# boguszjelinski/taxidispatcher

Measured on AMD Instinct MI355X. Metric: NxN assignments/sec, higher is better.
Workload: dtype int32; 1 GPU; g1 N=16384: device cost write (4N^2 B) + exact assignment, total checked == optimum; n=16384, parallelism=single GPU

## Files before the change

taxidispatcher_amd/csrc/td_assign.hip:

```cpp
#include <dlfcn.h>
#include <limits.h>
#include <stdlib.h>

#include <type_traits>

#include "td_common.h"

using namespace td;

namespace {

template <typename CT>
struct Tr;
template <>
struct Tr<uint8_t> {
    using PT = int32_t;
    static constexpr int E = 16;
    static constexpr uint32_t SENT = 0xFFu;
    static constexpr int64_t LIMIT = 254;
    static constexpr int32_t BIG = 1 << 28;
    static constexpr int32_t KMAX = INT32_MAX;
};
template <>
struct Tr<uint16_t> {
// ... 3094 lines not shown
            k_compress_tr<8><<<dim3((n + 63) / 64, (n + 511) / 512), 256, 0, c.stream>>>(n, npad, sv.d_cost, (uint32_t *)sv.cc.p, 0, colmin, colmax, ctl);
        else
            k_compress_tr<1><<<dim3((n + 63) / 64, (n + 63) / 64), 256, 0, c.stream>>>(n, npad, sv.d_cost, (uint32_t *)sv.cc.p, 0, colmin, colmax, ctl);
        k_tr_finish<<<(n + 255) / 256, 256, 0, c.stream>>>(n, 0, colmin, colmax, (int32_t *)sv.rowmin.p, (int *)sv.rconst.p, ctl, esc_raw,
                                                           cells8 ? 1 : 0, nosync ? (long long)assumed_range : -1ll);
    }
    TD_HIP(hipGetLastError());
    if (nosync) {
        *fits = true;
        sv.nconst = -1;
        sv.nchunks = nchunks;
        sv.npad = npad;
        return TD_OK;
    }
    TD_HIP(hipMemcpyAsync(c.pinned, ctl, 8 * sizeof(int), hipMemcpyDeviceToHost, c.stream));
    TD_HIP(hipStreamSynchronize(c.stream));
    const int *h = (const int *)c.pinned;
    *range = (int64_t)(((const unsigned long long *)(h + CTL_RANGE))[0]);
    *fits = h[CTL_FLAG] == 0 && *range <= (int64_t)Tr<uint32_t>::LIMIT && *range >= 0;
    sv.nconst = h[CTL_NCONST];
    if (*fits) {
        sv.nchunks = nchunks;
        sv.npad = npad;
    }
    return TD_OK;
}

int sv_complete_cc(Solver &sv)
{
    if (!sv.cc_partial) return TD_OK;
    Ctx &c = ctx();
    ProfScope ps(TD_K_COMPRESS);
    k_compress_rest<<<std::max(1, std::min(sv.nrows, c.n_cu * 8)), 256, 0, c.stream>>>(sv.n, sv.nrows, sv.row0, sv.nchunks, sv.cc_rpb, sv.d_cost,
                                                                                      (uint8_t *)sv.cc.p, (const int32_t *)sv.rowmin.p,
                                                                                      (const int *)sv.misc.p);
    TD_HIP(hipGetLastError());
    sv.cc_partial = false;
    return TD_OK;
}

template <typename CT>
int sv_hop_t(Solver &sv, int rpb, int ncols_blk, int col_lo, int nb, bool window_zero, uint8_t *ob, bool raw = false, bool gate = false)
{
    Ctx &c = ctx();
    using PT = typename Tr<CT>::PT;
    int rc;
    if ((rc = ensure(sv.esc, sizeof(unsigned long long) * 2 * (size_t)std::max(sv.nrows, 1)))) return rc;
    if ((rc = ensure(sv.hop, sizeof(HopCtl)))) return rc;
    if ((rc = ensure(sv.hoptab, sizeof(int) * (size_t)nb * HOP_FMAX * HOP_FMAX))) return rc;
    HopCtl *hc = (HopCtl *)sv.hop.p;
    int *frl = (int *)sv.list.p, *fcl = (int *)sv.pred.p;
    const int *ctl = (const int *)sv.misc.p;
    if (gate && nb != 1) return fail(TD_EINTERNAL, "a gated two-hop pass takes one block");
    k_hop_lists<<<nb, 1024, 0, c.stream>>>(rpb, ncols_blk, col_lo, (const int *)sv.r2c.p, (const int *)sv.owner.p, frl, fcl, hc, ctl,
                                           gate ? g_hop_max_rows : 0);
    if (raw) {
        if (!sv.d_cost || sv.n % 4) return fail(TD_EINVAL, "two-hop pass on the int32 matrix: no matrix, or n %% 4 != 0");
        k_hop_esc<CT, true><<<(sv.nrows + 3) / 4, 256, 0, c.stream>>>(sv.nrows, sv.n / 4, rpb, ncols_blk, col_lo, g_hop_max_rows,
                                                                      (const CT *)sv.d_cost, (const PT *)sv.price.p, (const int *)sv.r2c.p, fcl,
                                                                      hc, (unsigned long long *)sv.esc.p, ctl, (const int32_t *)sv.rowmin.p);
        k_hop_table<CT, true><<<nb * HOP_FMAX, 256, 0, c.stream>>>(sv.n, sv.nrows, sv.row0, sv.n / 4, rpb, ncols_blk, col_lo, g_hop_max_rows,
                                                                   window_zero ? 1 : 0, (const CT *)sv.d_cost, (const PT *)sv.price.p,
                                                                   (const int *)sv.owner.p, frl, hc, (const unsigned long long *)sv.esc.p,
                                                                   (int *)sv.hoptab.p, ctl, (const int32_t *)sv.rowmin.p);
    } else {
    k_hop_esc<CT><<<(sv.nrows + 3) / 4, 256, 0, c.stream>>>(sv.nrows, sv.nchunks, rpb, ncols_blk, col_lo, g_hop_max_rows, (const CT *)sv.cc.p,
                                                            (const PT *)sv.price.p, (const int *)sv.r2c.p, fcl, hc,
                                                            (unsigned long long *)sv.esc.p, ctl);
    k_hop_table<CT><<<nb * HOP_FMAX, 256, 0, c.stream>>>(sv.n, sv.nrows, sv.row0, sv.nchunks, rpb, ncols_blk, col_lo, g_hop_max_rows,
                                                         window_zero ? 1 : 0, (const CT *)sv.cc.p, (const PT *)sv.price.p,
                                                         (const int *)sv.owner.p, frl, hc, (const unsigned long long *)sv.esc.p,
                                                         (int *)sv.hoptab.p, ctl);
    }
    k_hop_match<PT><<<nb, HOP_FMAX, sizeof(uint32_t) * (size_t)((rpb + 31) / 32), c.stream>>>(
        sv.nrows, sv.row0, rpb, ncols_blk, col_lo, g_hop_max_rows, (PT *)sv.price.p, (int *)sv.owner.p, (int *)sv.r2c.p, ob, frl, fcl, hc,
        (const int *)sv.hoptab.p, (int *)sv.misc.p);
    TD_HIP(hipGetLastError());
    return TD_OK;
}

template <typename CT>
int sv_begin_t(Solver &sv);

int sv_phase_a(Solver &sv, int hop_passes)
{
    Ctx &c = ctx();
    const int n = sv.n, nrows = sv.nrows;
    const int rpb = n / sv.zs_V, nb = nrows / rpb;
    const int col_lo = (sv.row0 / rpb) * rpb, col_hi = col_lo + nb * rpb;
    int rc;
    if ((rc = ensure(sv.ob, (size_t)sv.npad + 64))) return rc;
    if (!sv.ob_clear) TD_HIP(hipMemsetAsync(sv.ob.p, 0, (size_t)sv.npad, c.stream));
    sv.ob_clear = false;
    ProfScope ps(TD_K_BID);
    int *ctl = (int *)sv.misc.p;
    const int ga = (col_hi - col_lo + 255) / 256;
    unsigned long long *bid = (unsigned long long *)sv.bid.p;
    auto assign = [&]() {
        k_zs_assign<<<ga, 256, 0, c.stream>>>(col_lo, col_hi, nrows, sv.row0, bid, (int32_t *)sv.price.p, (int *)sv.owner.p, (int *)sv.r2c.p,
                                              (uint8_t *)sv.ob.p, ctl);
    };
    if (sv.zs_round0) {
        if (!sv.began && (rc = sv_begin_t<uint8_t>(sv))) return rc;
        k_zs_bid<<<std::min(nrows, c.n_cu * 16), 256, 0, c.stream>>>(nrows, sv.row0, sv.nchunks, rpb, (const uint8_t *)sv.cc.p,
                                                                     (const uint8_t *)sv.ob.p, (const int *)sv.r2c.p, bid, ctl, 0, 0);
        sv.zs_round0 = false;
    }
    assign();
    for (int r = 1; r <= g_zs_rounds; r++) {
        k_zs_bid<<<std::min(nrows, c.n_cu * 16), 256, 0, c.stream>>>(nrows, sv.row0, sv.nchunks, rpb, (const uint8_t *)sv.cc.p,
                                                                     (const uint8_t *)sv.ob.p, (const int *)sv.r2c.p, bid, ctl, r, g_tie_evict);
        assign();
    }
    TD_HIP(hipGetLastError());
    for (int p = 0; p < hop_passes; p++)
        if ((rc = sv_hop_t<uint8_t>(sv, rpb, rpb, col_lo, nb, true, (uint8_t *)sv.ob.p))) return rc;
    if (getenv("TD_DEBUG") && hop_passes > 0) {
        HopCtl h;
        TD_HIP(hipMemcpyAsync(&h, sv.hop.p, sizeof(h), hipMemcpyDeviceToHost, c.stream));
        TD_HIP(hipStreamSynchronize(c.stream));
        fprintf(stderr, "[td] phase A: %d blocks of %d rows, %d local rounds; free rows / columns per block before the last two-hop pass:", nb, rpb, g_zs_rounds);
        for (int b = 0; b < nb; b++) fprintf(stderr, " %d/%d", h.nfr[b], h.nfc[b]);
        fprintf(stderr, " | matched %d, left %d\n", h.matched, h.left);
    }
    sv.zs_done = false;
    sv.bid0_done = false;
    sv.state_ready = true;
// ... 1716 lines not shown
```

taxidispatcher_amd/csrc/td_blocks.h:

```cpp


struct HopCtl {
    int nfr[HOP_BMAX], nfc[HOP_BMAX];
    int left;
    int matched;
    int pad[2];
};

__device__ __forceinline__ uint32_t zs_zero_bytes(uint32_t w)
{
    return ~(((w & 0x7F7F7F7Fu) + 0x7F7F7F7Fu) | w | 0x7F7F7F7Fu);
}

__global__ __launch_bounds__(256) void k_zs_bid(int nrows, int row0, int nchunks, int rpb, const uint8_t *__restrict__ cc,
                                                const uint8_t *__restrict__ ob, const int *__restrict__ r2c,
                                                unsigned long long *__restrict__ bid, const int *__restrict__ ctl, int round,
                                                int tie_evict)
{
    __shared__ int s_best[4];
    if (ctl[CTL_FLAG]) return;
    const int tid = threadIdx.x, lane = tid & 63, w = tid >> 6;
    const int cpb = rpb >> 4;
    const size_t pitch = (size_t)nchunks * 16;
    for (int lrow = blockIdx.x; lrow < nrows; lrow += gridDim.x) {
// ... 9 lines not shown
            if (ch >= cpb) ch -= cpb;
            ch += c0;
            const uint4 cv = *reinterpret_cast<const uint4 *>(rp + (size_t)ch * 16);
            const uint4 ov = *reinterpret_cast<const uint4 *>(ob + (size_t)ch * 16);
            const uint32_t cw[4] = {cv.x, cv.y, cv.z, cv.w}, ow[4] = {ov.x, ov.y, ov.z, ov.w};
#pragma unroll
            for (int k = 0; k < 4; k++) {
                const uint32_t z = zs_zero_bytes(cw[k]);
                if (!z) continue;
                const uint32_t zf = z & zs_zero_bytes(ow[k]);
                const uint32_t pick = zf ? zf : z;
                const int cand = (zf ? 0 : (1 << 24)) | (t * 16 + k * 4 + (__builtin_ctz(pick) >> 3));
                best = min(best, cand);
            }
        }
#pragma unroll
        for (int o = 32; o > 0; o >>= 1) best = min(best, __shfl_xor(best, o));
        if (lane == 0) s_best[w] = best;
        __syncthreads();
        if (tid == 0) {
            best = min(min(s_best[0], s_best[1]), min(s_best[2], s_best[3]));
            if (best != INT_MAX) {
                const bool owned = (best >> 24) != 0;
                const int pos = best & 0xFFFFFF;
                int ch = (pos >> 4) + rot;
                if (ch >= cpb) ch -= cpb;
                const int j = (c0 + ch) * 16 + (pos & 15);
                if (!owned || tie_evict) atomicMax(&bid[j], (unsigned long long)(row + 1));
            }
        }
        __syncthreads();
    }
}

__global__ __launch_bounds__(256) void k_zs_assign(int col_lo, int col_hi, int nrows, int row0, unsigned long long *__restrict__ bid,
                                                   int32_t *__restrict__ pk, int *__restrict__ owner, int *__restrict__ r2c,
                                                   uint8_t *__restrict__ ob, const int *__restrict__ ctl)
{
    if (ctl[CTL_FLAG]) return;
    const int j = col_lo + blockIdx.x * blockDim.x + threadIdx.x;
    if (j >= col_hi) return;
    const unsigned long long k = bid[j];
    if (!k) return;
    const int row = (int)(k & ((1ull << ROW_BITS) - 1)) - 1;
    const int old = owner[j];
    if (old >= row0 && old < row0 + nrows) r2c[old - row0] = -1;
    owner[j] = row;
    if (row >= row0 && row < row0 + nrows) r2c[row - row0] = j;
    pk[j] = 1;
    ob[j] = 1;
    bid[j] = 0ull;
}

__global__ __launch_bounds__(1024) void k_hop_lists(int rpb, int ncols_blk, int col_lo, const int *__restrict__ r2c,
                                                    const int *__restrict__ owner, int *__restrict__ frl, int *__restrict__ fcl,
                                                    HopCtl *__restrict__ hc, const int *__restrict__ ctl, int gate_max = 0)
{
    if (ctl[CTL_FLAG]) return;
    const int lb = blockIdx.x;
    if (gate_max > 0) {
        __shared__ int s_go;
        if (threadIdx.x == 0) {
            const int left = hc->left;
            s_go = left > 0 && left <= gate_max;
        }
        __syncthreads();
        if (!s_go) {
            if (threadIdx.x == 0) hc->nfr[lb] = 0, hc->nfc[lb] = 0;
            return;
        }
    }
    const int nfr = build_free_list(rpb, r2c + (size_t)lb * rpb, frl + (size_t)lb * rpb, -1);
    const int nfc = build_free_list(ncols_blk, owner + col_lo + (size_t)lb * ncols_blk, fcl + (size_t)lb * ncols_blk, -1);
    if (threadIdx.x == 0) {
        hc->nfr[lb] = nfr;
        hc->nfc[lb] = nfc;
        if (lb == 0) hc->left = 0, hc->matched = 0;
    }
}

template <typename CT, bool RAW = false>
__global__ __launch_bounds__(256) void k_hop_esc(int nrows, int nchunks, int rpb, int ncols_blk, int col_lo, int max_rows,
                                                 const CT *__restrict__ cc, const typename Tr<CT>::PT *__restrict__ pk,
                                                 const int *__restrict__ r2c, const int *__restrict__ fcl,
                                                 const HopCtl *__restrict__ hc, unsigned long long *__restrict__ esc,
                                                 const int *__restrict__ ctl, const int32_t *__restrict__ rowmin = nullptr)
{
    using PT = typename Tr<CT>::PT;
    if (ctl[CTL_FLAG]) return;
    const int lane = threadIdx.x & 63;
    const int lrow = blockIdx.x * 4 + (threadIdx.x >> 6);
    if (lrow >= nrows) return;
    const int lb = lrow / rpb;
    const int nfr = hc->nfr[lb];
    if (nfr == 0 || nfr > max_rows) return;
    const int nfc = min(hc->nfc[lb], HOP_FMAX);
    const int j = r2c[lrow];
    unsigned long long m0 = 0, m1 = 0;
    if (j >= 0) {
        const size_t pitch = (size_t)nchunks * (RAW ? 4 : Tr<CT>::E);
        const CT *rp = cc + (RAW ? 0 : (size_t)lrow * pitch);
        const int32_t *rr = reinterpret_cast<const int32_t *>(cc) + (RAW ? (size_t)lrow * pitch : 0);
        const int32_t mn = RAW ? rowmin[lrow] : 0;
        auto cell = [&](int col) -> long long {
            if constexpr (RAW) return (long long)(uint32_t)(rr[col] - mn);
            else return (long long)(uint32_t)rp[col];
        };
        const long long u = cell(j) + (long long)(pk[j] >> 1);
        const int *fc = fcl + (size_t)lb * ncols_blk;
        const int cb = col_lo + lb * ncols_blk;
        bool t0 = false, t1 = false;
        if (lane < nfc) {
            const int jb = cb + fc[lane];
            t0 = cell(jb) + (long long)(pk[jb] >> 1) == u;
        }
        if (lane + 64 < nfc) {
            const int jb = cb + fc[lane + 64];
            t1 = cell(jb) + (long long)(pk[jb] >> 1) == u;
        }
        m0 = __ballot(t0);
        m1 = __ballot(t1);
    }
    if (lane == 0) {
        esc[(size_t)lrow * 2] = m0;
        esc[(size_t)lrow * 2 + 1] = m1;
    }
}

template <typename CT, bool RAW = false>
__global__ __launch_bounds__(256) void k_hop_table(int n, int nrows, int row0, int nchunks, int rpb, int ncols_blk, int col_lo,
                                                   int max_rows, int window_zero, const CT *__restrict__ cc,
                                                   const typename Tr<CT>::PT *__restrict__ pk, const int *__restrict__ owner,
                                                   const int *__restrict__ frl, const HopCtl *__restrict__ hc,
                                                   const unsigned long long *__restrict__ esc, int *__restrict__ tab,
                                                   const int *__restrict__ ctl, const int32_t *__restrict__ rowmin = nullptr)
{
    using PT = typename Tr<CT>::PT;
    constexpr int E = RAW ? 4 : Tr<CT>::E;
    __shared__ int s_tab[HOP_FMAX];
    constexpr int CHT = RAW ? 4 : 1;
    __shared__ int s_cand[256 * E * CHT];
    __shared__ int s_ncand;
    __shared__ long long s_v[4];
    if (ctl[CTL_FLAG]) return;
    const int lb = blockIdx.x / HOP_FMAX, a = blockIdx.x % HOP_FMAX;
    const int nfr = hc->nfr[lb];
    if (nfr > max_rows || a >= min(nfr, HOP_FMAX)) return;
    const int tid = threadIdx.x, lane = tid & 63, w = tid >> 6;
    const int lrow = lb * rpb + frl[(size_t)lb * rpb + a];
    const size_t pitch = (size_t)nchunks * E;
    const unsigned char *rp = reinterpret_cast<const unsigned char *>(cc) + (size_t)lrow * pitch * (RAW ? 4 : sizeof(CT));
    const int32_t mn = RAW ? rowmin[lrow] : 0;
    auto cells = [&](const uint4 &raw, uint32_t *c) {
        if constexpr (RAW) {
            c[0] = (uint32_t)((int32_t)raw.x - mn), c[1] = (uint32_t)((int32_t)raw.y - mn);
            c[2] = (uint32_t)((int32_t)raw.z - mn), c[3] = (uint32_t)((int32_t)raw.w - mn);
        } else
            unpack<CT>(raw, c);
    };
    if (tid < HOP_FMAX) s_tab[tid] = INT_MAX;
    if (tid == 0) s_ncand = 0;
    const int ch_lo = window_zero ? (col_lo + lb * ncols_blk) / E : 0;
    const int ch_n = window_zero ? (ncols_blk + E - 1) / E : nchunks;
    long long v = 0;
    if (!window_zero) {
        long long mv = LLONG_MAX;
        for (int t = tid; t < ch_n; t += 256) {
            uint32_t c[E];
            cells(*reinterpret_cast<const uint4 *>(rp + (size_t)(ch_lo + t) * 16), c);
            PT pv[E];
            const int j0 = (ch_lo + t) * E;
            if constexpr (sizeof(PT) == 4) {
                const int4 *pp = reinterpret_cast<const int4 *>(pk + j0);
#pragma unroll
                for (int q = 0; q < E / 4; q++) {
                    const int4 x = pp[q];
                    pv[4 * q + 0] = x.x, pv[4 * q + 1] = x.y, pv[4 * q + 2] = x.z, pv[4 * q + 3] = x.w;
                }
            } else {
#pragma unroll
                for (int e = 0; e < E; e++) pv[e] = pk[j0 + e];
            }
#pragma unroll
            for (int e = 0; e < E; e++)
                if (j0 + e < n) mv = min(mv, (long long)c[e] + (long long)(pv[e] >> 1));
        }
#pragma unroll
        for (int o = 32; o > 0; o >>= 1) {
            const long long ov = __shfl_xor(mv, o);
            mv = ov < mv ? ov : mv;
        }
        if (lane == 0) s_v[w] = mv;
        __syncthreads();
        v = min(min(s_v[0], s_v[1]), min(s_v[2], s_v[3]));
    }
    __syncthreads();
    for (int t0 = 0; t0 < ch_n; t0 += 256 * CHT) {
        uint4 raws[CHT];
#pragma unroll
        for (int u = 0; u < CHT; u++) {
            const int t = t0 + u * 256 + tid;
            if (t < ch_n) raws[u] = *reinterpret_cast<const uint4 *>(rp + (size_t)(ch_lo + t) * 16);
        }
#pragma unroll
        for (int u = 0; u < CHT; u++) {
        const int t = t0 + u * 256 + tid;
        if (t < ch_n) {
            const uint4 raw = raws[u];
            bool any = true;
            if constexpr (!RAW && sizeof(CT) == 1 && std::is_same<CT, uint8_t>::value)
                if (window_zero) any = (zs_zero_bytes(raw.x) | zs_zero_bytes(raw.y) | zs_zero_bytes(raw.z) | zs_zero_bytes(raw.w)) != 0;
            if (any) {
                uint32_t c[E];
                cells(raw, c);
                PT pv[E];
                const int j0 = (ch_lo + t) * E;
                if constexpr (sizeof(PT) == 4) {
                    const int4 *pp = reinterpret_cast<const int4 *>(pk + j0);
#pragma unroll
                    for (int q = 0; q < E / 4; q++) {
                        const int4 x = pp[q];
                        pv[4 * q + 0] = x.x, pv[4 * q + 1] = x.y, pv[4 * q + 2] = x.z, pv[4 * q + 3] = x.w;
                    }
                } else {
#pragma unroll
                    for (int e = 0; e < E; e++) pv[e] = pk[j0 + e];
                }
#pragma unroll
                for (int e = 0; e < E; e++) {
                    const bool tight = j0 + e < n && (long long)c[e] + (long long)(pv[e] >> 1) == v && (!window_zero || c[e] == 0);
                    if (tight) s_cand[atomicAdd(&s_ncand, 1)] = j0 + e;
                }
            }
        }
        }
        __syncthreads();
        const int nc = s_ncand;
        for (int k = tid; k < nc; k += 256) {
            const int r = owner[s_cand[k]];
            if (r < row0 || r >= row0 + nrows) continue;
            if ((r - row0) / rpb != lb) continue;
            unsigned long long m0 = esc[(size_t)(r - row0) * 2], m1 = esc[(size_t)(r - row0) * 2 + 1];
            while (m0) {
                const int b = __builtin_ctzll(m0);
                m0 &= m0 - 1;
                atomicMin(&s_tab[b], r);
            }
            while (m1) {
                const int b = 64 + __builtin_ctzll(m1);
                m1 &= m1 - 1;
                atomicMin(&s_tab[b], r);
            }
        }
        __syncthreads();
        if (tid == 0) s_ncand = 0;
        __syncthreads();
    }
    if (tid < HOP_FMAX) tab[((size_t)lb * HOP_FMAX + a) * HOP_FMAX + tid] = s_tab[tid] == INT_MAX ? -1 : s_tab[tid];
}

template <typename PT>
__global__ __launch_bounds__(HOP_FMAX) void k_hop_match(int nrows, int row0, int rpb, int ncols_blk, int col_lo, int max_rows,
                                                        PT *__restrict__ pk, int *__restrict__ owner, int *__restrict__ r2c,
                                                        uint8_t *__restrict__ ob, const int *__restrict__ frl,
                                                        const int *__restrict__ fcl, HopCtl *__restrict__ hc,
                                                        const int *__restrict__ tab, int *__restrict__ ctl)
{
    extern __shared__ uint32_t s_usedr[];
    __shared__ int s_usedc[HOP_FMAX];
    __shared__ int s_key[2][2];
    if (ctl[CTL_FLAG]) return;
    const int lb = blockIdx.x;
    const int nfr = hc->nfr[lb];
    const int tid = threadIdx.x, lane = tid & 63, w = tid >> 6;
    if (nfr == 0) return;
    if (nfr > max_rows) {
        if (tid == 0) atomicAdd(&hc->left, nfr);
        return;
    }
    const int na = min(nfr, HOP_FMAX), nc = min(hc->nfc[lb], HOP_FMAX);
    for (int k = tid; k < (rpb + 31) / 32; k += HOP_FMAX) s_usedr[k] = 0u;
    s_usedc[tid] = 0;
    __syncthreads();
    const int *fr = frl + (size_t)lb * rpb, *fc = fcl + (size_t)lb * ncols_blk;
    const int blk_row0 = row0 + lb * rpb;
    const int my_fc = tid < nc ? fc[tid] : 0;
    int done = 0;
    int r_nx = tid < nc ? tab[((size_t)lb * HOP_FMAX + 0) * HOP_FMAX + tid] : -1;
    int i_nx = blk_row0 + fr[0];
    for (int a = 0; a < na; a++) {
        const int r = r_nx, i_g = i_nx;
        if (a + 1 < na) {
            r_nx = tid < nc ? tab[((size_t)lb * HOP_FMAX + a + 1) * HOP_FMAX + tid] : -1;
            i_nx = blk_row0 + fr[a + 1];
        }
        const uint32_t hsh = ((uint32_t)i_g + 1u) * 0x9E3779B1u;
        const int st = nc ? (int)(((uint64_t)(hsh ^ (hsh >> 15)) * (uint64_t)nc) >> 32) : 0;
        int key = INT_MAX;
        if (r >= 0 && !s_usedc[tid]) {
            const int rb = r - blk_row0;
            if (!((s_usedr[rb >> 5] >> (rb & 31)) & 1u)) {
                int t = tid - st;
                t += t < 0 ? nc : 0;
                key = t;
            }
        }
        int best = key;
#pragma unroll
        for (int o = 32; o > 0; o >>= 1) best = min(best, __shfl_xor(best, o));
        if (lane == 0) s_key[a & 1][w] = best;
        __syncthreads();
        best = min(s_key[a & 1][0], s_key[a & 1][1]);
        if (best != INT_MAX && key == best) {
            const int rl = r - row0, il = i_g - row0;
            const int j = r2c[rl], jp = col_lo + lb * ncols_blk + my_fc;
            r2c[il] = j;
            owner[j] = i_g;
            r2c[rl] = jp;
            owner[jp] = r;
            pk[jp] = pk[jp] | (PT)1;
            if (ob) ob[jp] = 1;
            s_usedc[tid] = 1;
            const int rb = r - blk_row0;
            atomicOr(&s_usedr[rb >> 5], 1u << (rb & 31));
        }
        if (best != INT_MAX) done++;
        __syncthreads();
    }
    if (tid == 0) {
        atomicAdd(&hc->left, nfr - done);
        atomicAdd(&hc->matched, done);
    }
}

__global__ void k_zs_owned_bits(int n, const int *__restrict__ owner, int32_t *__restrict__ pk)
{
    const int j = blockIdx.x * blockDim.x + threadIdx.x;
    if (j < n) pk[j] = (pk[j] & ~1) | (owner[j] >= 0 ? 1 : 0);
}
```

taxidispatcher_amd/csrc/td_line.hip:

```cpp
#include <limits.h>

#include <hipcub/hipcub.hpp>

#include "td_common.h"

namespace td {
namespace {

enum { LC_P = 0, LC_Q, LC_I1, LC_I2, LC_PLAUS, LC_REV, LC_FAIL, LC_FITS32, LC_TOTAL, LC_K, LC_FILL, LC_SKIP, LC_WORDS };
constexpr int LINE_KMAX = 256;

struct LineWs {
    Buf ctl, kin, kout, vin, vout, tmp, f, v64, v32, r2c;
    Buf band, P, E, ARG, Bk, L, mcol;
};
LineWs g_lw;

typedef int v4i __attribute__((ext_vector_type(4)));

struct ArgMax {
    long long v;
    int i;
};
__device__ inline bool better(const ArgMax &a, const ArgMax &b) { return a.v > b.v || (a.v == b.v && a.i < b.i); }

__device__ ArgMax block_argmax(ArgMax x, ArgMax *sh)
{
    const int lane = threadIdx.x & 63, w = threadIdx.x >> 6, nw = blockDim.x >> 6;
#pragma unroll
    for (int o = 32; o > 0; o >>= 1) {
        ArgMax y;
        y.v = __shfl_xor(x.v, o);
        y.i = __shfl_xor(x.i, o);
        if (better(y, x)) x = y;
    }
    __syncthreads();
    if (lane == 0) sh[w] = x;
    __syncthreads();
    ArgMax r = sh[0];
    for (int k = 1; k < nw; k++)
        if (better(sh[k], r)) r = sh[k];
    return r;
}

__device__ inline long long labs64(long long x) { return x < 0 ? -x : x; }

__device__ inline bool span_ok(long long x, long long y, long long D) { return x + y == D || labs64(x - y) == D; }

__global__ __launch_bounds__(1024) void k_line_probe(int n, const int32_t *__restrict__ c, long long *__restrict__ ctl,
                                                     long long *__restrict__ host_verdict, int *__restrict__ clear_words = nullptr,
                                                     int nclear = 0)
{
    for (int k = threadIdx.x; k < nclear; k += blockDim.x) clear_words[k] = 0;
    __shared__ ArgMax sh[16];
    __shared__ int s_cnt;
    const int t = threadIdx.x, T = blockDim.x;
    const int p = 0, i1 = 0;
    const int step = n > 1024 ? n / 1024 : 1;
    const int nsamp = (n + step - 1) / step;
    const long long u0 = c[0], w0 = c[n];
    const long long Ea = u0 + w0, Eb = labs64(u0 - w0);
    const long long B0 = c[(size_t)(n - 1) * n], B1 = c[n - 1];
    int mode = 0, rev = 0, q = -1, rq = 0, i2 = -1, kdummy = 0;
    int bad_a = 0, bad_b = 0, rowvar = 0, colvar = 0, far = 0;
    if (t == 0) s_cnt = 0;
    if (t < n) {
        const long long xx = c[t], yy = c[(size_t)n + t];
        bad_a = !span_ok(xx, yy, Ea);
        bad_b = !span_ok(xx, yy, Eb);
        rowvar = c[(size_t)(n - 1) * n + t] != B0;
        far = labs64(xx - u0) > 254;
    }
    if (t < nsamp) colvar = c[(size_t)(t * step) * n + (n - 1)] != B1;
    bad_a = __syncthreads_or(bad_a);
    bad_b = __syncthreads_or(bad_b);
    const bool rows_dummy = !__syncthreads_or(rowvar);
    const bool cols_dummy = !__syncthreads_or(colvar);
    const int far_any = __syncthreads_or(far);
    const int suspicious = far_any || cols_dummy;
    int est_cc = 0, est_cr = 0;
    if (cols_dummy) {
        const int step4 = n > 256 ? n / 256 : 1;
        const int ns4 = (n + step4 - 1) / step4;
        int ccol = 0, crow = 0;
        if (t < ns4) {
            const int j = t * step4, i = t * step4;
            const int32_t v0 = c[j], w0r = c[(size_t)i * n];
            int same_c = 1, same_r = 1;
#pragma unroll
            for (int k = 1; k < 8; k++) {
                const size_t kk = (size_t)(((long long)k * n) >> 3);
                same_c &= c[kk * n + j] == v0;
                same_r &= c[(size_t)i * n + kk] == w0r;
            }
            ccol = same_c;
            crow = same_r;
        }
        est_cc = __syncthreads_count(ccol) * step4;
        est_cr = __syncthreads_count(crow) * step4;
    }
    if (cols_dummy) {
        __shared__ int s_r, s_c1;
        if (t == 0) {
            s_r = INT_MAX;
// ... 84 lines not shown
                    cols_ok = !(bad_a && bad_b);
                }
            }
        }
        if (cols_ok && q >= 0 && i2 >= 0) {
            const long long x0 = c[(size_t)rq * n + p], y0 = c[(size_t)rq * n + q];
            const long long Da = x0 + y0, Db = labs64(x0 - y0);
            bad_a = bad_b = 0;
            for (int k = t; k < nsamp; k += T) {
                const int32_t *row = c + (size_t)(k * step) * n;
                const long long xx = row[p], yy = row[q];
                if (rows_dummy && xx == B0 && yy == B0) continue;
                bad_a |= !span_ok(xx, yy, Da);
                bad_b |= !span_ok(xx, yy, Db);
            }
            bad_a = __syncthreads_or(bad_a);
            bad_b = __syncthreads_or(bad_b);
            mode = !(bad_a && bad_b);
            if (mode && rows_dummy) {
                int cnt = 0;
                for (int i = t; i < n; i += T) cnt += c[(size_t)i * n + p] == B0 && c[(size_t)i * n + q] == B0;
#pragma unroll
                for (int o = 32; o > 0; o >>= 1) cnt += __shfl_xor(cnt, o);
                if ((t & 63) == 0 && cnt) atomicAdd(&s_cnt, cnt);
                __syncthreads();
                kdummy = s_cnt;
                mode = (kdummy >= 1 && kdummy <= LINE_KMAX && n - kdummy >= 2) ? 3 : 0;
            }
            const long long a1 = c[(size_t)i1 * n + p], b1 = c[(size_t)i1 * n + q], a2 = c[(size_t)i2 * n + p], b2 = c[(size_t)i2 * n + q];
            rev = (a2 * a2 - b2 * b2) < (a1 * a1 - b1 * b1);
        }
    }
    if (t == 0) {
        ctl[LC_P] = p;
        ctl[LC_Q] = q < 0 ? 0 : q;
        ctl[LC_I1] = i1;
        ctl[LC_I2] = i2 < 0 ? 0 : i2;
        ctl[LC_PLAUS] = mode;
        ctl[LC_REV] = rev;
        ctl[LC_FAIL] = mode == 0;
        ctl[LC_FITS32] = 0;
        ctl[LC_TOTAL] = 0;
        ctl[LC_K] = kdummy;
        ctl[LC_FILL] = B0;
        ctl[LC_SKIP] = (mode != 0 || suspicious) ? 1 : 0;
        host_verdict[3] = est_cc;
        host_verdict[4] = est_cr;
        host_verdict[5] = far_any;
        host_verdict[6] = B1;
        host_verdict[0] = mode;
        host_verdict[1] = kdummy;
        host_verdict[2] = suspicious;
        __threadfence_system();
    }
}

__global__ __launch_bounds__(256) void k_line_keys(int n, const int32_t *__restrict__ c, const long long *__restrict__ ctl,
                                                   unsigned long long *__restrict__ keys, int *__restrict__ vals)
{
    const int p = (int)ctl[LC_P], q = (int)ctl[LC_Q], i1 = (int)ctl[LC_I1], i2 = (int)ctl[LC_I2];
    const bool rev = ctl[LC_REV] != 0;
    const bool unbal = ctl[LC_PLAUS] == 3;
    const long long fill = ctl[LC_FILL];
    for (int t = blockIdx.x * blockDim.x + threadIdx.x; t < 2 * n; t += gridDim.x * blockDim.x) {
        long long x, y;
        if (t < n) {
            x = c[(size_t)t * n + p];
            y = c[(size_t)t * n + q];
            if (unbal && x == fill && y == fill) {
                keys[t] = 0x7fffffffffffffffull;
                vals[t] = t;
                continue;
            }
        } else {
            x = c[(size_t)i1 * n + (t - n)];
            y = c[(size_t)i2 * n + (t - n)];
        }
        long long key = x * x - y * y;
        if (t >= n && rev) key = -key;
        keys[t] = (unsigned long long)(key + (1ll << 62)) | (t < n ? 0ull : 1ull << 63);
        vals[t] = t < n ? t : t - n;
    }
}

__global__ __launch_bounds__(256) void k_line_gather(int n, const int32_t *__restrict__ c, const int *__restrict__ sorted,
                                                     long long *__restrict__ ctl, long long *__restrict__ f, int *__restrict__ r2c)
{
    __shared__ long long sh[4];
    const int *sig = sorted, *tau = sorted + n;
    long long sum = 0;
    int bad = 0;
    for (int k = blockIdx.x * blockDim.x + threadIdx.x; k < n; k += gridDim.x * blockDim.x) {
        const int s = sig[k], tk = tau[k];
        const int32_t *row = c + (size_t)s * n;
        const long long ckk = row[tk];
        long long d = 0;
        if (k + 1 < n) {
            const int tk1 = tau[k + 1];
            const int32_t *row1 = c + (size_t)sig[k + 1] * n;
            d = (long long)row[tk1] - ckk;
            const long long b = (long long)row1[tk] - (long long)row1[tk1];
            bad |= d + b < 0;
        }
        f[k] = d;
        r2c[s] = tk;
        sum += ckk;
// ... 415 lines not shown
            if (rev) key = -key;
            keys[t] = (unsigned long long)(key + (1ll << 62)) | 1ull << 63;
            vals[t] = t - n;
        }
    }
}

__global__ __launch_bounds__(256) void k_lsh_inv(int n, const int *__restrict__ sorted, int *__restrict__ inv, int *__restrict__ r2c)
{
    for (int k = blockIdx.x * blockDim.x + threadIdx.x; k < n; k += gridDim.x * blockDim.x) {
        inv[sorted[k]] = k;
        r2c[sorted[k]] = sorted[n + k];
    }
}

__global__ __launch_bounds__(256) void k_lsh_diffs(int n, int row0, int nrows, const int32_t *__restrict__ c, const int *__restrict__ sorted,
                                                   const int *__restrict__ inv, long long *__restrict__ F, long long *__restrict__ B,
                                                   long long *__restrict__ tot)
{
    __shared__ long long sh[4];
    const int *tau = sorted + n;
    long long sum = 0;
    for (int t = blockIdx.x * blockDim.x + threadIdx.x; t < nrows; t += gridDim.x * blockDim.x) {
        const int k = inv[row0 + t];
        const int32_t *row = c + (size_t)t * n;
        const long long ckk = row[tau[k]];
        if (k + 1 < n) F[k] = (long long)row[tau[k + 1]] - ckk;
        if (k > 0) B[k - 1] = (long long)row[tau[k - 1]] - ckk;
        sum += ckk;
    }
#pragma unroll
    for (int o = 32; o > 0; o >>= 1) sum += __shfl_xor(sum, o);
    if ((threadIdx.x & 63) == 0) sh[threadIdx.x >> 6] = sum;
    __syncthreads();
    if (threadIdx.x == 0) {
        sum = sh[0] + sh[1] + sh[2] + sh[3];
        if (sum) atomicAdd((unsigned long long *)tot, (unsigned long long)sum);
    }
}

__global__ __launch_bounds__(256) void k_lsh_monge(int n, const long long *__restrict__ F, const long long *__restrict__ B,
                                                   long long *__restrict__ ctl)
{
    int bad = ctl[LC_PLAUS] == 0;
    for (int k = blockIdx.x * blockDim.x + threadIdx.x; k + 1 < n; k += gridDim.x * blockDim.x) bad |= F[k] + B[k] < 0;
    if (bad) ctl[LC_FAIL] = 1;
}

__global__ void k_lsh_publish(const long long *__restrict__ ctl, long long *__restrict__ failw) { *failw = ctl[LC_FAIL] != 0; }

}

constexpr size_t VERDICT_OFF = 4096;
hipEvent_t g_probe_done = nullptr;

int line_probe_launch(int n, const int32_t *d_cost, const long long **skip_dev, int *clear_words, int nclear)
{
    Ctx &c = ctx();
    int rc;
    if ((rc = ensure(g_lw.ctl, 256))) return rc;
    if (!g_probe_done) TD_HIP(hipEventCreateWithFlags(&g_probe_done, hipEventDisableTiming));
    long long *ctl = (long long *)g_lw.ctl.p;
    {
        ProfScope ps(TD_K_LINE);
        k_line_probe<<<1, 1024, 0, c.stream>>>(n, d_cost, ctl, (long long *)((char *)c.pinned + VERDICT_OFF), clear_words,
                                               clear_words ? nclear : 0);
        TD_HIP(hipGetLastError());
    }
    TD_HIP(hipEventRecord(g_probe_done, c.stream));
    *skip_dev = ctl + LC_SKIP;
    return TD_OK;
}

int line_probe_wait(int *mode, int *k, int *suspicious, int *shape3)
{
    Ctx &c = ctx();
    TD_HIP(hipEventSynchronize(g_probe_done));
    const volatile long long *h = (const volatile long long *)((char *)c.pinned + VERDICT_OFF);
    *mode = (int)h[0];
    *k = (int)h[1];
    if (suspicious) *suspicious = (int)h[2];
    if (shape3) {
        shape3[0] = (int)h[3];
        shape3[1] = (int)h[4];
        shape3[2] = (int)h[5];
        shape3[3] = (int)h[6];
    }
    return TD_OK;
}

int line_finish(int n, int k, const int32_t *d_cost, const int32_t **r2c_dev, int64_t *total, int *accepted)
{
    Ctx &c = ctx();
    *accepted = 0;
    int rc;
    const size_t np = (size_t)n + 16;
    if ((rc = ensure(g_lw.kin, 16 * np))) return rc;
    if ((rc = ensure(g_lw.kout, 16 * np))) return rc;
    if ((rc = ensure(g_lw.vin, 8 * np))) return rc;
    if ((rc = ensure(g_lw.vout, 8 * np))) return rc;
    if ((rc = ensure(g_lw.f, 8 * np))) return rc;
    if ((rc = ensure(g_lw.v64, 8 * np))) return rc;
    if ((rc = ensure(g_lw.v32, 4 * np))) return rc;
    if ((rc = ensure(g_lw.r2c, 4 * np))) return rc;
    long long *ctl = (long long *)g_lw.ctl.p;
    auto *kin = (unsigned long long *)g_lw.kin.p, *kout = (unsigned long long *)g_lw.kout.p;
    int *vin = (int *)g_lw.vin.p, *vout = (int *)g_lw.vout.p;
    {
        ProfScope ps(TD_K_LINE);
        k_line_keys<<<std::max(1, std::min(c.n_cu * 4, (2 * n + 255) / 256)), 256, 0, c.stream>>>(n, d_cost, ctl, kin, vin);
        size_t bytes = 0;
        TD_HIP(hipcub::DeviceRadixSort::SortPairs(nullptr, bytes, kin, kout, vin, vout, 2 * n, 0, 64, c.stream));
        if ((rc = ensure(g_lw.tmp, bytes + 256))) return rc;
        TD_HIP(hipcub::DeviceRadixSort::SortPairs(g_lw.tmp.p, bytes, kin, kout, vin, vout, 2 * n, 0, 64, c.stream));
        if (k == 0) {
            k_line_gather<<<std::max(1, std::min(c.n_cu * 4, (n + 255) / 256)), 256, 0, c.stream>>>(n, d_cost, vout, ctl, (long long *)g_lw.f.p,
                                                                                                (int *)g_lw.r2c.p);
            k_line_scan<<<1, 1024, 0, c.stream>>>(n, vout, ctl, (const long long *)g_lw.f.p, (long long *)g_lw.v64.p, (int32_t *)g_lw.v32.p);
        } else {
            const size_t n1 = (size_t)n + 1;
            if ((rc = ensure(g_lw.band, 8 * (size_t)(k + 1) * n1))) return rc;
            if ((rc = ensure(g_lw.P, 8 * (size_t)(k + 1) * n1))) return rc;
            if ((rc = ensure(g_lw.ARG, 8 * (size_t)k * n1))) return rc;
            if ((rc = ensure(g_lw.E, 8 * n1))) return rc;
            if ((rc = ensure(g_lw.Bk, 8 * n1))) return rc;
            if ((rc = ensure(g_lw.L, 8 * n1))) return rc;
            if ((rc = ensure(g_lw.mcol, 4 * n1))) return rc;
            k_line_band<<<std::max(1, std::min(c.n_cu * 4, (int)(((size_t)(k + 1) * n + 255) / 256))), 256, 0, c.stream>>>(
                n, k, d_cost, vout, (long long *)g_lw.band.p);
            k_line_unbal<<<1, 1024, 0, c.stream>>>(n, k, d_cost, vout, ctl, (const long long *)g_lw.band.p, (long long *)g_lw.P.p,
                                                    (long long *)g_lw.E.p, (long long *)g_lw.ARG.p, (long long *)g_lw.f.p,
                                                    (long long *)g_lw.Bk.p, (long long *)g_lw.L.p, (int *)g_lw.mcol.p,
                                                    (long long *)g_lw.v64.p, (int32_t *)g_lw.v32.p, (int *)g_lw.r2c.p);
        }
        TD_HIP(hipGetLastError());
    }
    {
        ProfScope ps(TD_K_CERT);
        constexpr int R = 4;
        const int ngroups = (n + R - 1) / R;
        const int grid = std::max(1, std::min(ngroups, c.n_cu * 16));
        const bool vec = (n % 4 == 0) && (((uintptr_t)d_cost & 15) == 0);
        if (vec)
            k_line_cert<R, true><<<grid, 256, 0, c.stream>>>(n, n, d_cost, (const long long *)g_lw.v64.p, (const int32_t *)g_lw.v32.p,
                                                             (const int *)g_lw.r2c.p, ctl);
        else
            k_line_cert<R, false><<<grid, 256, 0, c.stream>>>(n, n, d_cost, (const long long *)g_lw.v64.p, (const int32_t *)g_lw.v32.p,
                                                              (const int *)g_lw.r2c.p, ctl);
        TD_HIP(hipGetLastError());
    }
    TD_HIP(hipMemcpyAsync(c.pinned, ctl, LC_WORDS * sizeof(long long), hipMemcpyDeviceToHost, c.stream));
    TD_HIP(hipStreamSynchronize(c.stream));
    const long long *h = (const long long *)c.pinned;
    if (h[LC_FAIL] == 0) {
        *accepted = 1;
        *total = h[LC_TOTAL];
        *r2c_dev = (const int32_t *)g_lw.r2c.p;
    }
    return TD_OK;
}

void line_release_workspace()
{
    if (g_probe_done) (void)hipEventDestroy(g_probe_done);
    g_probe_done = nullptr;
    Buf *bs[] = {&g_lw.ctl, &g_lw.kin,  &g_lw.kout, &g_lw.vin, &g_lw.vout, &g_lw.tmp, &g_lw.f,  &g_lw.v64, &g_lw.v32,
                 &g_lw.r2c, &g_lw.band, &g_lw.P,    &g_lw.E,   &g_lw.ARG,  &g_lw.Bk,  &g_lw.L,  &g_lw.mcol};
    for (Buf *b : bs) buf_free(*b);
}

}

using namespace td;

extern "C" int64_t td_line_shard_ws_words(int n) { return n < 2 ? 0 : (int64_t)LshLayout(n).end; }

extern "C" int td_line_shard_phase(int phase, int n, int row0, int nrows, const int32_t *cost_rows, int64_t *ws, int64_t *seg_off,
                                   int64_t *seg_len)
{
    TD_REQUIRE_INIT();
    Ctx &c = ctx();
    if (n < 2 || row0 < 0 || nrows < 0 || (long long)row0 + nrows > n) return fail(TD_EINVAL, "td_line_shard_phase: bad shard %d+%d of %d", row0, nrows, n);
    if (!ws || !seg_off || !seg_len) return fail(TD_EINVAL, "td_line_shard_phase: null argument");
    if (nrows > 0 && (!cost_rows || !is_device_ptr(cost_rows))) return fail(TD_EINVAL, "td_line_shard_phase: cost_rows must be device memory");
    if (!is_device_ptr(ws)) return fail(TD_EINVAL, "td_line_shard_phase: ws must be device memory");
    const LshLayout L(n);
    long long *w = (long long *)ws, *ctl = w + L.ctl;
    const int grid_rows = std::max(1, std::min(c.n_cu * 4, (nrows + 255) / 256));
    const int grid_n = std::max(1, std::min(c.n_cu * 4, (2 * n + 255) / 256));
    int rc;
    ProfScope ps(phase == 3 ? TD_K_CERT : TD_K_LINE);
    switch (phase) {
    case 0:
        TD_HIP(hipMemsetAsync(w, 0, L.end * 8, c.stream));
        if (row0 == 0 && nrows > 0) k_lsh_anchor<<<1, 1024, 0, c.stream>>>(n, nrows, cost_rows, ctl, (int32_t *)(w + L.anch), L.N2);
        *seg_off = 0, *seg_len = (int64_t)(L.anch + L.N2);
        break;
    case 1:
        if (nrows > 0) k_lsh_rowkeys<<<grid_rows, 256, 0, c.stream>>>(n, row0, nrows, cost_rows, ctl, w + L.rk);
        *seg_off = (int64_t)L.rk, *seg_len = n;
        break;
    case 2: {
        auto *kin = (unsigned long long *)(w + L.kin), *kout = (unsigned long long *)(w + L.kout);
        int *vin = (int *)(w + L.vin), *sorted = (int *)(w + L.sorted);
        k_lsh_keys<<<grid_n, 256, 0, c.stream>>>(n, ctl, (const int32_t *)(w + L.anch), L.N2, w + L.rk, kin, vin);
        size_t bytes = 0;
        TD_HIP(hipcub::DeviceRadixSort::SortPairs(nullptr, bytes, kin, kout, vin, sorted, 2 * n, 0, 64, c.stream));
        if ((rc = ensure(g_lw.tmp, bytes + 256))) return rc;
        TD_HIP(hipcub::DeviceRadixSort::SortPairs(g_lw.tmp.p, bytes, kin, kout, vin, sorted, 2 * n, 0, 64, c.stream));
        k_lsh_inv<<<grid_n, 256, 0, c.stream>>>(n, sorted, (int *)(w + L.inv), (int *)(w + L.r2c));
        if (nrows > 0)
            k_lsh_diffs<<<grid_rows, 256, 0, c.stream>>>(n, row0, nrows, cost_rows, sorted, (const int *)(w + L.inv), w + L.fb, w + L.fb + L.N2,
                                                         w + L.tot);
        *seg_off = (int64_t)L.fb, *seg_len = (int64_t)(2 * L.N2 + 1);
        break;
    }
    case 3: {
        k_lsh_monge<<<grid_n, 256, 0, c.stream>>>(n, w + L.fb, w + L.fb + L.N2, ctl);
// ... 43 lines not shown
```

Baseline: 27.62 million assignments/s.

## Split two-hop table over column segments, wave-level matching, spin-poll line probe verdict

For raw int32 windowed two-hop passes, the table kernel is split across several column segments per row. Each segment writes global atomicMin results into a table that k_hop_lists presets, instead of a per-block shared table. The match kernel now loads the whole table into LDS and runs the greedy matching in a single wavefront using ballots and readlane, with no per-row block barriers. Commits are then applied in parallel at the end. Separately, the line probe wait replaces hipEventSynchronize with a host spin on a sequence number written to pinned memory, with a timeout fallback; this trades host CPU spinning and added global atomics for lower latency.

New measurement: 28.97 million assignments/s (median of 6 runs). 4.9% higher.

```diff
diff --git a/taxidispatcher_amd/csrc/td_assign.hip b/taxidispatcher_amd/csrc/td_assign.hip
--- a/taxidispatcher_amd/csrc/td_assign.hip
+++ b/taxidispatcher_amd/csrc/td_assign.hip
@@ -3170,13 +3170,19 @@
     int *frl = (int *)sv.list.p, *fcl = (int *)sv.pred.p;
     const int *ctl = (const int *)sv.misc.p;
     if (gate && nb != 1) return fail(TD_EINTERNAL, "a gated two-hop pass takes one block");
+    const int nseg = raw && window_zero ? (ncols_blk / 4 + 1023) / 1024 : 1;
     k_hop_lists<<<nb, 1024, 0, c.stream>>>(rpb, ncols_blk, col_lo, (const int *)sv.r2c.p, (const int *)sv.owner.p, frl, fcl, hc, ctl,
-                                           gate ? g_hop_max_rows : 0);
+                                           gate ? g_hop_max_rows : 0, nseg > 1 ? (int *)sv.hoptab.p : nullptr);
     if (raw) {
         if (!sv.d_cost || sv.n % 4) return fail(TD_EINVAL, "two-hop pass on the int32 matrix: no matrix, or n %% 4 != 0");
         k_hop_esc<CT, true><<<(sv.nrows + 3) / 4, 256, 0, c.stream>>>(sv.nrows, sv.n / 4, rpb, ncols_blk, col_lo, g_hop_max_rows,
                                                                       (const CT *)sv.d_cost, (const PT *)sv.price.p, (const int *)sv.r2c.p, fcl,
                                                                       hc, (unsigned long long *)sv.esc.p, ctl, (const int32_t *)sv.rowmin.p);
+        if (nseg > 1)
+            k_hop_table<CT, true, true><<<nb * HOP_FMAX * nseg, 256, 0, c.stream>>>(
+                sv.n, sv.nrows, sv.row0, sv.n / 4, rpb, ncols_blk, col_lo, g_hop_max_rows, 1, (const CT *)sv.d_cost, (const PT *)sv.price.p,
+                (const int *)sv.owner.p, frl, hc, (const unsigned long long *)sv.esc.p, (int *)sv.hoptab.p, ctl, (const int32_t *)sv.rowmin.p, nseg);
+        else
         k_hop_table<CT, true><<<nb * HOP_FMAX, 256, 0, c.stream>>>(sv.n, sv.nrows, sv.row0, sv.n / 4, rpb, ncols_blk, col_lo, g_hop_max_rows,
                                                                    window_zero ? 1 : 0, (const CT *)sv.d_cost, (const PT *)sv.price.p,
                                                                    (const int *)sv.owner.p, frl, hc, (const unsigned long long *)sv.esc.p,
@@ -3190,7 +3196,10 @@
                                                          (const int *)sv.owner.p, frl, hc, (const unsigned long long *)sv.esc.p,
                                                          (int *)sv.hoptab.p, ctl);
     }
-    k_hop_match<PT><<<nb, HOP_FMAX, sizeof(uint32_t) * (size_t)((rpb + 31) / 32), c.stream>>>(
+    const size_t match_lds = sizeof(uint32_t) * ((size_t)HOP_FMAX * HOP_FMAX + (size_t)((rpb + 31) / 32));
+    if (match_lds > 150 * 1024) return fail(TD_EINVAL, "two-hop pass: a block of that many rows does not fit the LDS");
+    TD_HIP(hipFuncSetAttribute((const void *)k_hop_match<PT>, hipFuncAttributeMaxDynamicSharedMemorySize, (int)match_lds));
+    k_hop_match<PT><<<nb, HOP_MATCH_T, match_lds, c.stream>>>(
         sv.nrows, sv.row0, rpb, ncols_blk, col_lo, g_hop_max_rows, (PT *)sv.price.p, (int *)sv.owner.p, (int *)sv.r2c.p, ob, frl, fcl, hc,
         (const int *)sv.hoptab.p, (int *)sv.misc.p);
     TD_HIP(hipGetLastError());
diff --git a/taxidispatcher_amd/csrc/td_blocks.h b/taxidispatcher_amd/csrc/td_blocks.h
--- a/taxidispatcher_amd/csrc/td_blocks.h
+++ b/taxidispatcher_amd/csrc/td_blocks.h
@@ -85,9 +85,11 @@
     bid[j] = 0ull;
 }
 
+constexpr int HOP_NONE = INT_MAX;
 __global__ __launch_bounds__(1024) void k_hop_lists(int rpb, int ncols_blk, int col_lo, const int *__restrict__ r2c,
                                                     const int *__restrict__ owner, int *__restrict__ frl, int *__restrict__ fcl,
-                                                    HopCtl *__restrict__ hc, const int *__restrict__ ctl, int gate_max = 0)
+                                                    HopCtl *__restrict__ hc, const int *__restrict__ ctl, int gate_max = 0,
+                                                    int *__restrict__ tab_preset = nullptr)
 {
     if (ctl[CTL_FLAG]) return;
     const int lb = blockIdx.x;
@@ -109,6 +111,10 @@
         hc->nfr[lb] = nfr;
         hc->nfc[lb] = nfc;
         if (lb == 0) hc->left = 0, hc->matched = 0;
+    }
+    if (tab_preset) {
+        int4 *t4 = reinterpret_cast<int4 *>(tab_preset + (size_t)lb * HOP_FMAX * HOP_FMAX);
+        for (int k = threadIdx.x; k < min(nfr, HOP_FMAX) * (HOP_FMAX / 4); k += 1024) t4[k] = make_int4(HOP_NONE, HOP_NONE, HOP_NONE, HOP_NONE);
     }
 }
 
@@ -160,13 +166,14 @@
     }
 }
 
-template <typename CT, bool RAW = false>
+template <typename CT, bool RAW = false, bool SPLIT = false>
 __global__ __launch_bounds__(256) void k_hop_table(int n, int nrows, int row0, int nchunks, int rpb, int ncols_blk, int col_lo,
                                                    int max_rows, int window_zero, const CT *__restrict__ cc,
                                                    const typename Tr<CT>::PT *__restrict__ pk, const int *__restrict__ owner,
                                                    const int *__restrict__ frl, const HopCtl *__restrict__ hc,
                                                    const unsigned long long *__restrict__ esc, int *__restrict__ tab,
-                                                   const int *__restrict__ ctl, const int32_t *__restrict__ rowmin = nullptr)
+                                                   const int *__restrict__ ctl, const int32_t *__restrict__ rowmin = nullptr,
+                                                   int nseg = 1)
 {
     using PT = typename Tr<CT>::PT;
     constexpr int E = RAW ? 4 : Tr<CT>::E;
@@ -176,7 +183,8 @@
     __shared__ int s_ncand;
     __shared__ long long s_v[4];
     if (ctl[CTL_FLAG]) return;
-    const int lb = blockIdx.x / HOP_FMAX, a = blockIdx.x % HOP_FMAX;
+    const int seg = SPLIT ? (int)blockIdx.x % nseg : 0, ba = SPLIT ? (int)blockIdx.x / nseg : (int)blockIdx.x;
+    const int lb = ba / HOP_FMAX, a = ba % HOP_FMAX;
     const int nfr = hc->nfr[lb];
     if (nfr > max_rows || a >= min(nfr, HOP_FMAX)) return;
     const int tid = threadIdx.x, lane = tid & 63, w = tid >> 6;
@@ -191,7 +199,8 @@
         } else
             unpack<CT>(raw, c);
     };
-    if (tid < HOP_FMAX) s_tab[tid] = INT_MAX;
+    int *tab_row = tab + ((size_t)lb * HOP_FMAX + a) * HOP_FMAX;
+    if (!SPLIT && tid < HOP_FMAX) s_tab[tid] = INT_MAX;
     if (tid == 0) s_ncand = 0;
     const int ch_lo = window_zero ? (col_lo + lb * ncols_blk) / E : 0;
     const int ch_n = window_zero ? (ncols_blk + E - 1) / E : nchunks;
@@ -228,7 +237,7 @@
         v = min(min(s_v[0], s_v[1]), min(s_v[2], s_v[3]));
     }
     __syncthreads();
-    for (int t0 = 0; t0 < ch_n; t0 += 256 * CHT) {
+    for (int t0 = SPLIT ? seg * 256 * CHT : 0; t0 < (SPLIT ? min(ch_n, (seg + 1) * 256 * CHT) : ch_n); t0 += 256 * CHT) {
         uint4 raws[CHT];
 #pragma unroll
         for (int u = 0; u < CHT; u++) {
@@ -274,95 +283,130 @@
             if (r < row0 || r >= row0 + nrows) continue;
             if ((r - row0) / rpb != lb) continue;
             unsigned long long m0 = esc[(size_t)(r - row0) * 2], m1 = esc[(size_t)(r - row0) * 2 + 1];
+            int *dst = SPLIT ? tab_row : s_tab;
             while (m0) {
                 const int b = __builtin_ctzll(m0);
                 m0 &= m0 - 1;
-                atomicMin(&s_tab[b], r);
+                atomicMin(&dst[b], r);
             }
             while (m1) {
                 const int b = 64 + __builtin_ctzll(m1);
                 m1 &= m1 - 1;
-                atomicMin(&s_tab[b], r);
+                atomicMin(&dst[b], r);
             }
         }
         __syncthreads();
         if (tid == 0) s_ncand = 0;
         __syncthreads();
     }
-    if (tid < HOP_FMAX) tab[((size_t)lb * HOP_FMAX + a) * HOP_FMAX + tid] = s_tab[tid] == INT_MAX ? -1 : s_tab[tid];
-}
-
+    if (!SPLIT && tid < HOP_FMAX) tab_row[tid] = s_tab[tid] == INT_MAX ? -1 : s_tab[tid];
+}
+
+constexpr int HOP_MATCH_T = 256;
 template <typename PT>
-__global__ __launch_bounds__(HOP_FMAX) void k_hop_match(int nrows, int row0, int rpb, int ncols_blk, int col_lo, int max_rows,
-                                                        PT *__restrict__ pk, int *__restrict__ owner, int *__restrict__ r2c,
-                                                        uint8_t *__restrict__ ob, const int *__restrict__ frl,
-                                                        const int *__restrict__ fcl, HopCtl *__restrict__ hc,
-                                                        const int *__restrict__ tab, int *__restrict__ ctl)
-{
-    extern __shared__ uint32_t s_usedr[];
-    __shared__ int s_usedc[HOP_FMAX];
-    __shared__ int s_key[2][2];
+__global__ __launch_bounds__(HOP_MATCH_T) void k_hop_match(int nrows, int row0, int rpb, int ncols_blk, int col_lo, int max_rows,
+                                                           PT *__restrict__ pk, int *__restrict__ owner, int *__restrict__ r2c,
+                                                           uint8_t *__restrict__ ob, const int *__restrict__ frl,
+                                                           const int *__restrict__ fcl, HopCtl *__restrict__ hc,
+                                                           const int *__restrict__ tab, int *__restrict__ ctl)
+{
+    extern __shared__ uint32_t s_hop_dyn[];
+    __shared__ int s_st[HOP_FMAX];
+    __shared__ int s_win[HOP_FMAX][2];
     if (ctl[CTL_FLAG]) return;
     const int lb = blockIdx.x;
     const int nfr = hc->nfr[lb];
-    const int tid = threadIdx.x, lane = tid & 63, w = tid >> 6;
+    const int tid = threadIdx.x;
     if (nfr == 0) return;
     if (nfr > max_rows) {
         if (tid == 0) atomicAdd(&hc->left, nfr);
         return;
     }
     const int na = min(nfr, HOP_FMAX), nc = min(hc->nfc[lb], HOP_FMAX);
-    for (int k = tid; k < (rpb + 31) / 32; k += HOP_FMAX) s_usedr[k] = 0u;
-    s_usedc[tid] = 0;
-    __syncthreads();
+    int *s_tab = reinterpret_cast<int *>(s_hop_dyn);
+    uint32_t *s_usedr = s_hop_dyn + HOP_FMAX * HOP_FMAX;
     const int *fr = frl + (size_t)lb * rpb, *fc = fcl + (size_t)lb * ncols_blk;
     const int blk_row0 = row0 + lb * rpb;
-    const int my_fc = tid < nc ? fc[tid] : 0;
-    int done = 0;
-    int r_nx = tid < nc ? tab[((size_t)lb * HOP_FMAX + 0) * HOP_FMAX + tid] : -1;
-    int i_nx = blk_row0 + fr[0];
-    for (int a = 0; a < na; a++) {
-        const int r = r_nx, i_g = i_nx;
-        if (a + 1 < na) {
-            r_nx = tid < nc ? tab[((size_t)lb * HOP_FMAX + a + 1) * HOP_FMAX + tid] : -1;
-            i_nx = blk_row0 + fr[a + 1];
-        }
-        const uint32_t hsh = ((uint32_t)i_g + 1u) * 0x9E3779B1u;
-        const int st = nc ? (int)(((uint64_t)(hsh ^ (hsh >> 15)) * (uint64_t)nc) >> 32) : 0;
-        int key = INT_MAX;
-        if (r >= 0 && !s_usedc[tid]) {
-            const int rb = r - blk_row0;
-            if (!((s_usedr[rb >> 5] >> (rb & 31)) & 1u)) {
-                int t = tid - st;
-                t += t < 0 ? nc : 0;
-                key = t;
-            }
-        }
-        int best = key;
-#pragma unroll
-        for (int o = 32; o > 0; o >>= 1) best = min(best, __shfl_xor(best, o));
-        if (lane == 0) s_key[a & 1][w] = best;
-        __syncthreads();
-        best = min(s_key[a & 1][0], s_key[a & 1][1]);
-        if (best != INT_MAX && key == best) {
-            const int rl = r - row0, il = i_g - row0;
-            const int j = r2c[rl], jp = col_lo + lb * ncols_blk + my_fc;
-            r2c[il] = j;
-            owner[j] = i_g;
-            r2c[rl] = jp;
-            owner[jp] = r;
-            pk[jp] = pk[jp] | (PT)1;
-            if (ob) ob[jp] = 1;
-            s_usedc[tid] = 1;
-            const int rb = r - blk_row0;
-            atomicOr(&s_usedr[rb >> 5], 1u << (rb & 31));
-        }
-        if (best != INT_MAX) done++;
-        __syncthreads();
-    }
-    if (tid == 0) {
-        atomicAdd(&hc->left, nfr - done);
-        atomicAdd(&hc->matched, done);
+    const int my_i = tid < na ? blk_row0 + fr[tid] : 0;
+    {
+        const int4 *src = reinterpret_cast<const int4 *>(tab + (size_t)lb * HOP_FMAX * HOP_FMAX);
+        int4 *dst = reinterpret_cast<int4 *>(s_tab);
+        auto norm = [&](int r, int col) { return (r == HOP_NONE || col >= nc) ? -1 : r; };
+        for (int k = tid; k < na * (HOP_FMAX / 4); k += HOP_MATCH_T) {
+            const int4 x = src[k];
+            const int col = (k * 4) & (HOP_FMAX - 1);
+            dst[k] = make_int4(norm(x.x, col), norm(x.y, col + 1), norm(x.z, col + 2), norm(x.w, col + 3));
+        }
+        for (int k = tid; k < (rpb + 31) / 32; k += HOP_MATCH_T) s_usedr[k] = 0u;
+        if (tid < na) {
+            const uint32_t hsh = ((uint32_t)my_i + 1u) * 0x9E3779B1u;
+            s_st[tid] = nc ? (int)(((uint64_t)(hsh ^ (hsh >> 15)) * (uint64_t)nc) >> 32) : 0;
+        }
+    }
+    __syncthreads();
+    if (tid < 64) {
+        const int lane = tid;
+        auto entry = [&](int a, int col) -> int {
+            const int r = s_tab[min(a, HOP_FMAX - 1) * HOP_FMAX + col];
+            return a < na ? r : -1;
+        };
+        auto used = [&](int r) -> bool {
+            const int rb = max(r - blk_row0, 0);
+            const uint32_t word = s_usedr[rb >> 5];
+            return r < 0 || ((word >> (rb & 31)) & 1u);
+        };
+        unsigned long long usedc0 = 0ull, usedc1 = 0ull;
+        int done = 0, r_prev = -1;
+        int ra0 = entry(0, lane), ra1 = entry(0, lane + 64);
+        int rb0 = entry(1, lane), rb1 = entry(1, lane + 64);
+        bool ua0 = used(ra0), ua1 = used(ra1);
+        int st = s_st[0];
+        for (int a = 0; a < na; a++) {
+            const int rc0 = entry(a + 2, lane), rc1 = entry(a + 2, lane + 64);
+            const bool ub0 = used(rb0), ub1 = used(rb1);
+            const int st_nx = s_st[min(a + 1, HOP_FMAX - 1)];
+            const unsigned long long m0 = __ballot(!ua0 && ra0 != r_prev) & ~usedc0;
+            const unsigned long long m1 = __ballot(!ua1 && ra1 != r_prev) & ~usedc1;
+            int rw = -1, cw = 0;
+            if (m0 | m1) {
+                const unsigned long long h0 = st < 64 ? m0 & (~0ull << st) : 0ull;
+                const unsigned long long h1 = st < 64 ? m1 : m1 & (~0ull << (st - 64));
+                if (h0 | h1) cw = h0 ? __builtin_ctzll(h0) : 64 + __builtin_ctzll(h1);
+                else cw = m0 ? __builtin_ctzll(m0) : 64 + __builtin_ctzll(m1);
+                rw = __builtin_amdgcn_readlane(cw < 64 ? ra0 : ra1, cw & 63);
+                if (cw < 64) usedc0 |= 1ull << cw;
+                else usedc1 |= 1ull << (cw - 64);
+                r_prev = rw;
+                done++;
+            }
+            if (lane == 0) {
+                s_win[a][0] = rw, s_win[a][1] = cw;
+                if (rw >= 0) {
+                    const int rb = rw - blk_row0;
+                    atomicOr(&s_usedr[rb >> 5], 1u << (rb & 31));
+                }
+            }
+            __builtin_amdgcn_fence(__ATOMIC_ACQ_REL, "wavefront");
+            ra0 = rb0, ra1 = rb1, ua0 = ub0, ua1 = ub1;
+            rb0 = rc0, rb1 = rc1;
+            st = st_nx;
+        }
+        if (lane == 0) {
+            atomicAdd(&hc->left, nfr - done);
+            atomicAdd(&hc->matched, done);
+        }
+    }
+    __syncthreads();
+    if (tid < na && s_win[tid][0] >= 0) {
+        const int r = s_win[tid][0], i_g = my_i;
+        const int rl = r - row0, il = i_g - row0;
+        const int j = r2c[rl], jp = col_lo + lb * ncols_blk + fc[s_win[tid][1]];
+        r2c[il] = j;
+        owner[j] = i_g;
+        r2c[rl] = jp;
+        owner[jp] = r;
+        pk[jp] = pk[jp] | (PT)1;
+        if (ob) ob[jp] = 1;
     }
 }
 
diff --git a/taxidispatcher_amd/csrc/td_line.hip b/taxidispatcher_amd/csrc/td_line.hip
--- a/taxidispatcher_amd/csrc/td_line.hip
+++ b/taxidispatcher_amd/csrc/td_line.hip
@@ -1,4 +1,5 @@
 #include <limits.h>
+#include <chrono>
 
 #include <hipcub/hipcub.hpp>
 
@@ -8,6 +9,7 @@
 namespace {
 
 enum { LC_P = 0, LC_Q, LC_I1, LC_I2, LC_PLAUS, LC_REV, LC_FAIL, LC_FITS32, LC_TOTAL, LC_K, LC_FILL, LC_SKIP, LC_WORDS };
+constexpr int VERDICT_SEQ = 7;
 constexpr int LINE_KMAX = 256;
 
 struct LineWs {
@@ -49,7 +51,7 @@
 
 __global__ __launch_bounds__(1024) void k_line_probe(int n, const int32_t *__restrict__ c, long long *__restrict__ ctl,
                                                      long long *__restrict__ host_verdict, int *__restrict__ clear_words = nullptr,
-                                                     int nclear = 0)
+                                                     int nclear = 0, long long seq = 0 )
 {
     for (int k = threadIdx.x; k < nclear; k += blockDim.x) clear_words[k] = 0;
     __shared__ ArgMax sh[16];
@@ -240,6 +242,7 @@
         host_verdict[1] = kdummy;
         host_verdict[2] = suspicious;
         __threadfence_system();
+        __hip_atomic_store(&host_verdict[VERDICT_SEQ], seq, __ATOMIC_RELEASE, __HIP_MEMORY_SCOPE_SYSTEM);
     }
 }
 
@@ -761,22 +764,22 @@
 }
 
 constexpr size_t VERDICT_OFF = 4096;
-hipEvent_t g_probe_done = nullptr;
+long long g_probe_seq = 0;
 
 int line_probe_launch(int n, const int32_t *d_cost, const long long **skip_dev, int *clear_words, int nclear)
 {
     Ctx &c = ctx();
     int rc;
     if ((rc = ensure(g_lw.ctl, 256))) return rc;
-    if (!g_probe_done) TD_HIP(hipEventCreateWithFlags(&g_probe_done, hipEventDisableTiming));
     long long *ctl = (long long *)g_lw.ctl.p;
+    long long *verdict = (long long *)((char *)c.pinned + VERDICT_OFF);
+    ((volatile long long *)verdict)[VERDICT_SEQ] = 0;
+    g_probe_seq++;
     {
         ProfScope ps(TD_K_LINE);
-        k_line_probe<<<1, 1024, 0, c.stream>>>(n, d_cost, ctl, (long long *)((char *)c.pinned + VERDICT_OFF), clear_words,
-                                               clear_words ? nclear : 0);
+        k_line_probe<<<1, 1024, 0, c.stream>>>(n, d_cost, ctl, verdict, clear_words, clear_words ? nclear : 0, g_probe_seq);
         TD_HIP(hipGetLastError());
     }
-    TD_HIP(hipEventRecord(g_probe_done, c.stream));
     *skip_dev = ctl + LC_SKIP;
     return TD_OK;
 }
@@ -784,8 +787,15 @@
 int line_probe_wait(int *mode, int *k, int *suspicious, int *shape3)
 {
     Ctx &c = ctx();
-    TD_HIP(hipEventSynchronize(g_probe_done));
     const volatile long long *h = (const volatile long long *)((char *)c.pinned + VERDICT_OFF);
+    const auto t0 = std::chrono::steady_clock::now();
+    while (__atomic_load_n((const long long *)&h[VERDICT_SEQ], __ATOMIC_ACQUIRE) != g_probe_seq) {
+        if (std::chrono::steady_clock::now() - t0 > std::chrono::milliseconds(20)) {
+            TD_HIP(hipStreamSynchronize(c.stream));
+            if (h[VERDICT_SEQ] != g_probe_seq) return fail(TD_EINTERNAL, "the line probe's verdict was not written");
+            break;
+        }
+    }
     *mode = (int)h[0];
     *k = (int)h[1];
     if (suspicious) *suspicious = (int)h[2];
@@ -871,8 +881,6 @@
 
 void line_release_workspace()
 {
-    if (g_probe_done) (void)hipEventDestroy(g_probe_done);
-    g_probe_done = nullptr;
     Buf *bs[] = {&g_lw.ctl, &g_lw.kin,  &g_lw.kout, &g_lw.vin, &g_lw.vout, &g_lw.tmp, &g_lw.f,  &g_lw.v64, &g_lw.v32,
                  &g_lw.r2c, &g_lw.band, &g_lw.P,    &g_lw.E,   &g_lw.ARG,  &g_lw.Bk,  &g_lw.L,  &g_lw.mcol};
     for (Buf *b : bs) buf_free(*b);
```
